# junghoseong/aircombat-selfplay

Hardware: AMD Instinct MI355X
Metric: agent-steps/sec (higher is better)
Workload: dtype f32

## Files before the change

### aircombat-selfplay_amd/csrc/aircombat.hip

```cpp
#include <hip/hip_runtime.h>
#include <stdint.h>
#include <stdio.h>
#include <string.h>
#include <string>
#include <vector>
#include <cmath>
#include <algorithm>
#include <chrono>
#include "../../include/aircombat.h"
#include "../../include/aircombat_buffer.h"
#include "clk_stamps.hpp"
#include "f16_device.hpp"
#include "f16_split.hpp"

using f16::State;
using f16::Derived;
using f16::Tab;
using f16::clampf;

#define AC_F_FIELDS(X)                                                                                           \
  X(vx) X(vy) X(vz) X(q0) X(q1) X(q2) X(q3) X(wp) X(wq) X(wr) X(hv1x) X(hv1y) X(hv1z) X(hv2x) X(hv2y) X(hv2z)   \
  X(ha1x) X(ha1y) X(ha1z) X(wdx) X(wdy) X(wdz) X(aix) X(aiy) X(aiz) X(bax) X(bay) X(baz) X(da) X(de) X(dr)       \
  X(thr) X(pin_r) X(pin_p) X(pin_y) X(pi_r) X(pi_p) X(pi_y) X(tef) X(ail) X(elev) X(sbdeg) X(alpha) X(mach)      \
  X(qc) X(vg) X(ap) X(aq) X(ar) X(npx) X(npy) X(npz) X(n1) X(n2) X(n2norm) X(ff) X(tank0) X(tank1)
// ... 734 lines not shown
    AC_CLKW(0, 120); AC_CLKW(1, 121); AC_CLKW(2, 122);
    __syncthreads();
  } else if (QUAD) {
    const int role = __builtin_amdgcn_readfirstlane(threadIdx.x >> 6);
    TableCopy<256> tc;
    tc.issue(P.tab);
    s = State{}; t = Task{};
    if (role == 0) { load_flight_role<0>(P.F, P.I, P.D, N, nn, s); t.status = state_word(P.F, SW_status, N, nn); }
    else if (role == 1) load_flight_role<1>(P.F, P.I, P.D, N, nn, s);
    else if (role == 2) { load_flight_role<2>(P.F, P.I, P.D, N, nn, s); t.status = state_word(P.F, SW_status, N, nn); }
    else {
      load_task(P.F, P.I, N, nn, t);
      s.ticks = state_word(P.F, SW_ticks, N, nn);
#pragma unroll
      for (int k = 0; k < MSLOTS; ++k) pre_st[k] = P.MI[((size_t)k * NMI + MI_status) * (size_t)N + nn];
    }
    __builtin_amdgcn_s_barrier();
    tc.write(lds_tab);
    a4 = make_float4(0.f, 0.f, 0.f, 0.f);
    __builtin_amdgcn_s_waitcnt(0x0F70);
    if (role == 1) arow.issue(act, c.act_dim);
    __syncthreads();
    if (role == 0) { quad_dynamics_wave(P, c, T, LQ, l, n, live, s, t); return; }
    if (role != 3 && split_helper_wave<true>(s, t, T, LQ.S, l, c.substeps, nullptr, nullptr, &arow)) return;
  } else if (PAIR) {
    const bool flight_role = __builtin_amdgcn_readfirstlane(threadIdx.x >> 6) == 1;
    PairFlightIn fin;
    if (!flight_role) {
      a4 = make_float4(0.f, 0.f, 0.f, 0.f);
      s = State{}; load_task(P.F, P.I, N, nn, t);
#pragma unroll
      for (int k = 0; k < MSLOTS; ++k) pre_st[k] = P.MI[((size_t)k * NMI + MI_status) * (size_t)N + nn];
    }
    stage_tables<128>(lds_tab, P.tab);
    if (flight_role) {
      pair_flight_load(P, c, nn, fin);
      pair_flight_wave<true>(P, c, T, LP, l, n, live, fin);
      return;
    }

  } else {
    TableCopy<64> tc;
    tc.issue(P.tab);
    a4 = load_controls(act, c.act_dim);
    if (TASK == AC_TASK_SHOOT_MISSILE) shoot_raw = act[4];
    load_state(P.F, P.I, P.D, N, nn, s, t);
    tc.commit(lds_tab);
  }
  AC_CLK(1);
  const Task was = t;
  constexpr bool OBS_BY_KIN = SPLIT && TASK == AC_TASK_SINGLECOMBAT;
  if (SPLIT) {
    const int role = __builtin_amdgcn_readfirstlane(threadIdx.x >> 6);
    if (split_helper_wave(s, t, T, L, l, c.substeps, nullptr, nullptr, &arow)) {
      if (OBS_BY_KIN && role == 1) {
        using namespace mail;
        wg_sync();
        Props q;
        q.alt_m = L.M[T_PR][l]; q.ub = L.M[T_PR + 5][l];
        q.n = L.M[T_PR + 9][l]; q.e = L.M[T_PR + 10][l]; q.u = L.M[T_PR + 11][l];
        q.vn = L.M[T_PR + 12][l]; q.ve = L.M[T_PR + 13][l]; q.vd = L.M[T_PR + 14][l];
        const Enemy Eq = exchange_1v1(q);
        L.M[T_RALT][l] = altitude_raw(q, c);
        L.M[T_RPOS][l] = posture_raw(q, Eq);
        wg_sync();
      }
      if (OBS_BY_KIN && role == 2) {
        using namespace mail;
        wg_sync();
        Props q;
        q.alt_m = L.M[T_PR][l]; q.sphi = L.M[T_PR + 1][l]; q.cphi = L.M[T_PR + 2][l]; q.stht = L.M[T_PR + 3][l]; q.ctht = L.M[T_PR + 4][l];
        q.ub = L.M[T_PR + 5][l]; q.vb = L.M[T_PR + 6][l]; q.wb = L.M[T_PR + 7][l]; q.vc = L.M[T_PR + 8][l];
        q.n = L.M[T_PR + 9][l]; q.e = L.M[T_PR + 10][l]; q.u = L.M[T_PR + 11][l];
        q.vn = L.M[T_PR + 12][l]; q.ve = L.M[T_PR + 13][l]; q.vd = L.M[T_PR + 14][l];
        const Enemy Eq = exchange_1v1(q);
        const Incoming none{false, 0, 0, 0, 0, 0, 0};
        float obq[OBS];
        observe_1v1<TASK>(q, Eq, none, obq);
        wg_sync();
        if (L.M[T_DONE][l] != 0.0f) {
          const float* tobs = (const float*)(P.tF + (size_t)NSW * 2) + slot * OBS;
#pragma unroll
          for (int k = 0; k < OBS; ++k) obq[k] = tobs[k];
        }
        float* row = lds_out + l * OBS;
#pragma unroll
        for (int k = 0; k < OBS; ++k) row[k] = obq[k];
        emit_obs_rows(P, lds_out, OBS, l);
      }
      return;
    }
  }
  Msl ms[MSLOTS];
  int nslots = 0, msl_was_active = 0;
  if (HAS_MSL) {
    nslots = min(c.num_missiles[slot], MSLOTS);
#pragma unroll
    for (int k = 0; k < MSLOTS; ++k) {
      const int st = (k < nslots) ? (PAIR ? pre_st[k] : P.MI[((size_t)k * NMI + MI_status) * (size_t)N + nn]) : MSL_INACTIVE;
      if (st != MSL_INACTIVE) { load_msl(P.MF, P.MI, N, nn, k, ms[k]); msl_was_active |= 1 << k; }
      else { ms[k] = Msl{}; ms[k].status = MSL_INACTIVE; }
    }
  }

  t.cur_step += 1;
  if (!SPLIT) {
    s.da = clampf(-1.0f, a4.x / 20.0f - 1.0f, 1.0f);
    s.de = clampf(-1.0f, a4.y / 20.0f - 1.0f, 1.0f);
    s.dr = clampf(-1.0f, a4.z / 20.0f - 1.0f, 1.0f);
    s.thr = clampf(0.0f, a4.w / 58.0f + 0.4f, 0.9f);
  }
  if (TASK == AC_TASK_SHOOT_MISSILE && !PAIR) t.shoot_action = (shoot_raw != 0.0f) ? 1 : 0;

  const MslParam MP = aim9l();
  bool have_pose = false;
  int last_tick = -1;
  bool env_has_missiles = false;
  if (PAIR) {
    bool mine = false;
#pragma unroll
    for (int k = 0; k < MSLOTS; ++k) mine = mine || ms[k].status != MSL_INACTIVE;
    const int other = __shfl_xor((int)mine, 1);
    env_has_missiles = mine || (bool)other;
  }
  int quad_nrun = 0;
  const int quad_ticks0 = s.ticks;
  for (int sub = 0; sub < c.substeps; ++sub) {
    bool fly_munitions = HAS_MSL;
    if (QUAD) {
      quad_substep_begin<true>(t, LQ, l, sub, env_has_missiles, quad_ticks0, quad_nrun, pr, c);
      fly_munitions = env_has_missiles;
    } else if (PAIR) {
      AC_CLK(2 + 8 * sub);
      pair_substep<true>(t, LP, l, sub, env_has_missiles, pr, c);
      AC_CLK(4 + 8 * sub);
      if (!env_has_missiles) continue;
    } else if (SPLIT) {
      if (dynamics_wave_tick(s, t, d, T, L, l, sub)) { have_pose = true; last_tick = sub; }
    } else if (t.status == AC_ALIVE) {
      if (t.bloods <= 0.0f) t.status = AC_SHOTDOWN;
      f16::tick<false>(s, d, T);
      have_pose = true;
    }
    if (HAS_MSL && fly_munitions) {
      if (!PAIR) {
      f16::locate(s, d);
      if (!have_pose) { f16::body_frame(s, d); have_pose = true; }
      make_props(s, d, c, pr);
      }
      float tx = __shfl_xor(pr.n, 1), ty = __shfl_xor(pr.e, 1), tz = __shfl_xor(pr.u, 1);
      float tvx = __shfl_xor(pr.vn, 1), tvy = __shfl_xor(pr.ve, 1), tvz = __shfl_xor(pr.vd, 1);
      bool talive = __shfl_xor(t.status, 1) == AC_ALIVE;
      bool hit_now = false;
#pragma unroll
      for (int k = 0; k < MSLOTS; ++k) {
        if (k < nslots && ms[k].status != MSL_INACTIVE) {
          missile_run(ms[k], MP, tx, ty, tz, tvx, tvy, tvz, talive, c);
          if (ms[k].status == MSL_HIT && talive) { hit_now = true; talive = false; }
        }
      }
      if (__shfl_xor((int)hit_now, 1) && t.status == AC_ALIVE) t.status = AC_SHOTDOWN;
      AC_CLK(5 + 8 * sub);
    }
    if (QUAD) wg_sync();
  }
  const bool split_located = SPLIT && dynamics_wave_finish(s, d, L, l, last_tick, c.substeps);
  if (PAIR) {
    if (QUAD) wg_sync();
    wg_sync();
    pair_read_final(LP, l, s, d, pr);
  } else if (!HAS_MSL || c.substeps == 0) {
    if (!split_located) f16::locate(s, d);
    if (!have_pose) f16::body_frame(s, d);
    make_props(s, d, c, pr);
  }
  AC_CLK(52);
  if (OBS_BY_KIN) {
    using namespace mail;
    L.M[T_PR][l] = pr.alt_m; L.M[T_PR + 1][l] = pr.sphi; L.M[T_PR + 2][l] = pr.cphi; L.M[T_PR + 3][l] = pr.stht; L.M[T_PR + 4][l] = pr.ctht;
    L.M[T_PR + 5][l] = pr.ub; L.M[T_PR + 6][l] = pr.vb; L.M[T_PR + 7][l] = pr.wb; L.M[T_PR + 8][l] = pr.vc;
    L.M[T_PR + 9][l] = pr.n; L.M[T_PR + 10][l] = pr.e; L.M[T_PR + 11][l] = pr.u;
    L.M[T_PR + 12][l] = pr.vn; L.M[T_PR + 13][l] = pr.ve; L.M[T_PR + 14][l] = pr.vd;
    wg_sync();
  }
  Enemy E = exchange_1v1(pr);

  if (c.use_artillery) {
    Geo g = ao_ta_r<false>(pr.n, pr.e, pr.u, pr.vn, pr.ve, pr.vd, E.n, E.e, E.u, E.vn, E.ve, E.vd);
    bool ealive = __shfl_xor(t.status, 1) == AC_ALIVE;
    float of = (g.AO <= 0.5236f) ? 1.0f - g.AO / 0.5236f : 0.0f;
    float Rk = g.R * 0.001f;
    float df = (Rk <= 1.0f) ? 1.0f : ((Rk <= 3.0f) ? (3.0f - Rk) * 0.5f : 0.0f);
    float dmg = ealive ? of * df : 0.0f;
    t.bloods -= __shfl_xor(dmg, 1);
  }
  if (HAS_MSL) {
    bool launch;
    if (TASK == AC_TASK_SHOOT_MISSILE && PAIR) t.shoot_action = ((QUAD ? LQ.S.M[mail::F_BITS][l] : LP.FIN[pair::FIN_BITS][l]) != 0.0f) ? 1 : 0;
    if (TASK == AC_TASK_DODGE_MISSILE) {
      const float dx = E.n - pr.n, dy = E.e - pr.e, dz = E.u - pr.u;
      const float dist = sqrtf(dx * dx + dy * dy + dz * dz);
      const float sp = sqrtf(pr.vn * pr.vn + pr.ve * pr.ve + pr.vd * pr.vd);
      const float ang = 57.29577951f * acosf(clampf(-1.0f, (dx * pr.vn + dy * pr.ve + dz * pr.vd) / (dist * sp + 1e-8f), 1.0f));
      const int len = c.lock_len;
      const unsigned bit = 1u << (unsigned)(t.lock_pos % len);
      t.lock_bits = (ang < c.max_attack_angle) ? (t.lock_bits | (int)bit) : (t.lock_bits & ~(int)bit);
      t.lock_pos += 1;
      const bool locked = __popc((unsigned)t.lock_bits & ((1u << len) - 1u)) >= len;
      launch = t.status == AC_ALIVE && locked && dist <= c.max_attack_distance && t.remaining > 0 &&
               (t.cur_step - t.last_shoot_time) >= c.min_attack_interval;
      if (launch) t.last_shoot_time = t.cur_step;
    } else {
      bool prev_done = t.last_missile < 0;
#pragma unroll
      for (int k = 0; k < MSLOTS; ++k)
        if (k == t.last_missile) prev_done = (ms[k].status == MSL_HIT || ms[k].status == MSL_MISS);
      launch = t.status == AC_ALIVE && t.shoot_action && t.remaining > 0 && prev_done;
    }
    int k = nslots - t.remaining;
// ... 1547 lines not shown
```

### aircombat-selfplay_amd/csrc/f16_split.hpp

```cpp
#pragma once

namespace f16 {
struct Surf { float aileron_rad, flaperon_rad, elevator_rad, rudder_rad, lef_rad, sb_rad, throttle_pos; };
struct DynVars {
  float gx, gy, gz;
  Atmos A;
  float mass, cgx, cgy, cgz, Jxx, Jyy, Jzz, Jxy, Jxz, Jyz;
  float vt, alpha, beta, ca, sa, cb, sb, qbar, mach, vg, qc, npx, npy, npz;
  float c00, c01, c02, c11, c12, c22, idet, im_;
  float bi2vel, ci2vel, qS, clb, cnb, cndr_m, kge;
  float4 g0, g1, g2, g3, ge, g7, m0, m1;
};
#define F16_DYN_REFS(k)                                                                                                          \
  float &gx = k.gx, &gy = k.gy, &gz = k.gz; Atmos& A = k.A;                                                                      \
  float &mass = k.mass, &cgx = k.cgx, &cgy = k.cgy, &cgz = k.cgz, &Jxx = k.Jxx, &Jyy = k.Jyy, &Jzz = k.Jzz, &Jxy = k.Jxy, &Jxz = k.Jxz, &Jyz = k.Jyz; \
  float &c00 = k.c00, &c01 = k.c01, &c02 = k.c02, &c11 = k.c11, &c12 = k.c12, &c22 = k.c22, &idet = k.idet, &im_ = k.im_; \
  float &vt = k.vt, &alpha = k.alpha, &beta = k.beta, &ca = k.ca, &sa = k.sa, &cb = k.cb, &sb = k.sb, &qbar = k.qbar, &mach = k.mach, &vg = k.vg,    \
        &qc = k.qc, &npx = k.npx, &npy = k.npy, &npz = k.npz;                                                                    \
  float &bi2vel = k.bi2vel, &ci2vel = k.ci2vel, &qS = k.qS, &clb = k.clb, &cnb = k.cnb, &cndr_m = k.cndr_m, &kge = k.kge; \
  float4 &g0 = k.g0, &g1 = k.g1, &g2 = k.g2, &g3 = k.g3, &ge = k.ge, &g7 = k.g7, &m0 = k.m0, &m1 = k.m1;                     \
  (void)gx; (void)gy; (void)gz; (void)A; (void)mass; (void)cgx; (void)cgy; (void)cgz; (void)Jxx; (void)Jyy; (void)Jzz; (void)Jxy; (void)Jxz; (void)Jyz; \
  (void)c00; (void)c01; (void)c02; (void)c11; (void)c12; (void)c22; (void)idet; (void)im_; \
  (void)vt; (void)alpha; (void)beta; (void)ca; (void)sa; (void)cb; (void)sb; (void)qbar; (void)mach; (void)vg; (void)qc; (void)npx; (void)npy; (void)npz; \
  (void)bi2vel; (void)ci2vel; (void)qS; (void)clb; (void)cnb; (void)cndr_m; (void)kge; (void)g0; (void)g1; (void)g2; (void)g3; (void)ge; (void)g7; (void)m0; (void)m1
// ... 179 lines not shown
    m1 = lerp4(rm2, rm3, fmach);
    cndr_m = lerpf(rn0, rn1, fmach);
    float hb = d.h_sl_ft * (1.0f / (float)F16_WINGSPAN);
    kge = 1.0f;
    if (hb < 1.1f) {
      constexpr float kGX[] = {0.0f, 0.1f, 0.15f, 0.2f, 0.3f, 0.4f, 0.5f, 0.6f, 0.7f, 0.8f, 0.9f, 1.0f, 1.1f};
      int ig = seg_index(kGX, hb);
      kge = lerpf(T[P_KCLGE_Y_OFF + ig - 1], T[P_KCLGE_Y_OFF + ig], seg_frac(T[P_KCLGE_X_OFF + ig - 1], T[P_KCLGE_X_OFF + ig], hb));
    }
  }
}

__device__ __forceinline__ void dyn_p4(State& s, Derived& d, DynVars& k, const Surf& sf, float thrust) {
  F16_DYN_REFS(k);
  const float aileron_rad = sf.aileron_rad, flaperon_rad = sf.flaperon_rad, rudder_rad = sf.rudder_rad, lef_rad = sf.lef_rad, sb_rad = sf.sb_rad;
  const float bw = (float)F16_WINGSPAN, cbar = (float)F16_CHORD;
  const float* Tb = d.T;
  (void)Tb;
  float tx = kInch2Ft * (cgx - (float)F16_THRUSTER_X), ty = kInch2Ft * ((float)F16_THRUSTER_Y - cgy), tz = kInch2Ft * (cgz - (float)F16_THRUSTER_Z);
  (void)tx;
  const float Mpy = tz * thrust, Mpz = -ty * thrust;

  float Fx, Fy, Fz, Mx, My, Mz;
  {
    float p = d.p, q = d.q, r = d.r;
    float qc = q * ci2vel;
    float CD = ge.x + m0.x + lef_rad * g0.x + flaperon_rad * (float)F16_K_CDDFLAPS + (float)F16_K_CDGEAR + sb_rad * g3.x +
               qc * (g0.y + lef_rad * g0.z);
    float CY = beta * ((float)F16_K_CYB + m0.y) + aileron_rad * (float)F16_K_CYDA + rudder_rad * (float)F16_K_CYDR +
               bi2vel * (p * g1.x + r * g1.y);
    float CL = kge * (ge.y + lef_rad * g0.w + flaperon_rad * (float)F16_K_CLDFLAPS + sb_rad * g3.y + qc * g2.x) + qc * sb_rad * g3.z;
    float Cl = clb + beta * m0.z + bi2vel * (p * g1.z + r * g1.w) + aileron_rad * (g7.x + alpha * m0.w) + rudder_rad * (g7.y + alpha * m1.x);
    float Cm = ge.z + alpha * m1.y + sb_rad * g3.w + qc * g2.y;
    float Cn = cnb + beta * m1.z + bi2vel * (p * g2.z + r * g2.w) + aileron_rad * (m1.w + g7.z) + rudder_rad * (g7.w + alpha * cndr_m);
    float D = qS * CD, Y = qS * CY, L = qS * CL;
    Fx = ca * cb * (-D) - ca * sb * Y + sa * L;
    Fy = sb * (-D) + cb * Y;
    Fz = sa * cb * (-D) - sa * sb * Y - ca * L;
    float ax = kInch2Ft * (cgx - (float)F16_AERORP_X), ay = kInch2Ft * ((float)F16_AERORP_Y - cgy), az = kInch2Ft * (cgz - (float)F16_AERORP_Z);
    Mx = qS * bw * Cl + (ay * Fz - az * Fy);
    My = qS * cbar * Cm + (az * Fx - ax * Fz);
    Mz = qS * bw * Cn + (ax * Fy - ay * Fx);
  }
  {
    float Tx = Fx + thrust, Ty = Fy, Tz = Fz;
    float Lm = Mx, Mm = My + Mpy, Nm = Mz + Mpz;
    float hx = Jxx * s.wp + Jxy * s.wq + Jxz * s.wr;
    float hy = Jxy * s.wp + Jyy * s.wq + Jyz * s.wr;
    float hz = Jxz * s.wp + Jyz * s.wq + Jzz * s.wr;
    float rx_ = Lm - (s.wq * hz - s.wr * hy), ry_ = Mm - (s.wr * hx - s.wp * hz), rz_ = Nm - (s.wp * hy - s.wq * hx);
    s.wdx = (c00 * rx_ + c01 * ry_ + c02 * rz_) * idet;
    s.wdy = (c01 * rx_ + c11 * ry_ + c12 * rz_) * idet;
    s.wdz = (c02 * rx_ + c12 * ry_ + c22 * rz_) * idet;
    s.bax = Tx * im_; s.bay = Ty * im_; s.baz = Tz * im_;
    s.aix = Tb[0] * s.bax + Tb[3] * s.bay + Tb[6] * s.baz + gx;
    s.aiy = Tb[1] * s.bax + Tb[4] * s.bay + Tb[7] * s.baz + gy;
    s.aiz = Tb[2] * s.bax + Tb[5] * s.bay + Tb[8] * s.baz + gz;
  }
  s.alpha = alpha; s.mach = mach; s.qc = qc; s.vg = vg;
  s.ap = d.p; s.aq = d.q; s.ar = d.r;
  s.npx = npx; s.npy = npy; s.npz = npz;
}

__device__ __forceinline__ void sys_fcs(State& s, float cthcph, float vbody, Surf& sf) {
  float &aileron_rad = sf.aileron_rad, &flaperon_rad = sf.flaperon_rad, &elevator_rad = sf.elevator_rad, &rudder_rad = sf.rudder_rad,
        &lef_rad = sf.lef_rad, &sb_rad = sf.sb_rad, &throttle_pos = sf.throttle_pos;
  const float alpha_p = s.alpha, mach_p = s.mach, qc_p = s.qc;
  float tef_rad = (qc_p < kQc250) ? 0.349f : ((mach_p > 0.9f) ? -0.0349f : 0.0f);
  s.tef = tef_kinematic(s.tef, 2.864789f * tef_rad);
  float roll_err = s.da - 0.31821f * s.ap;
  float roll_pid = pid(roll_err, s.pin_r, s.pi_r, qc_p < kQc20, 3.0f, 0.0005f, -0.00125f);
  float roll_cmd = clampf(-1.0f, roll_pid + s.da, 1.0f);
  aileron_rad = 0.375f * roll_cmd;
  s.ail = slew(s.ail, roll_cmd, -1.0f, 1.0f, 2.0f / 0.3f);
  constexpr float kAilX[] = C_FCS_AILERON_SPEED_COMPENSATED_X, kAilY[] = C_FCS_AILERON_SPEED_COMPENSATED_Y;
  float ail_sc = s.ail * tabc(kAilX, kAilY, mach_p);
  flaperon_rad = 1.4324f * (clampf(-1.0f, -s.tef - ail_sc, 1.0f) + clampf(-1.0f, s.tef - ail_sc, 1.0f));
  float elev_lim = clampf(-1.0f, s.de, 0.44f);
  constexpr float kElX[] = C_FCS_ELEVATOR_SCHEDULER_X, kElY[] = C_FCS_ELEVATOR_SCHEDULER_Y;
  float elev_sched = elev_lim * tabc(kElX, kElY, alpha_p);
  float pitch_err = elev_sched + 6.2f * s.aq - 0.020f * (s.npz - cthcph);
  float g_pid = clampf(-1.0f, pid(pitch_err, s.pin_p, s.pi_p, qc_p < kQc5, 0.3f, 0.025f, 0.0f), 1.0f);
  float pitch_sched = clampf(-1.0f, elev_sched + 1.0472f * alpha_p + g_pid, 1.0f);
  s.elev = slew(s.elev, pitch_sched, -1.0f, 1.0f, 2.0f / 0.3f);
  elevator_rad = 0.436f * s.elev;
  constexpr float kYwX[] = C_FCS_YAW_RATE_NORM_X, kYwY[] = C_FCS_YAW_RATE_NORM_Y;
  float yaw_err = s.dr + s.ar * tabc(kYwX, kYwY, s.vg) + 0.25f * s.npy;
  float yaw_pid = clampf(-1.0f, pid(yaw_err, s.pin_y, s.pi_y, qc_p < kQc10, 0.1055f, 0.00001f, 0.00005f), 1.0f);
  float yaw_sched = clampf(-1.0f, s.dr + yaw_pid, 1.0f);
  rudder_rad = 0.524f * slew(yaw_pid, yaw_sched, -1.0f, 1.0f, 2.0f / 0.4f);
  lef_rad = (alpha_p > 0.0873f) ? 0.262f : ((mach_p > 0.9f) ? -0.0349f : 0.0f);
  throttle_pos = 2.0f * s.thr;
  float sb_in = ((alpha_p * 57.29577951f >= 53.0f) && (vbody <= 18.0f)) ? 0.71667f * 60.0f : 0.0f;
  s.sbdeg = slew(s.sbdeg, sb_in, 0.0f, 60.0f, 60.0f);
  sb_rad = s.sbdeg * 0.01745329252f;

}

__device__ __forceinline__ void sys_mass(const State& s, DynVars& k) {
  F16_DYN_REFS(k);
  float fuel = s.tank0 + s.tank1;
  float weight = (float)F16_EMPTYWT + (float)F16_PM0_WEIGHT + fuel;
  mass = kLb2Slug * weight;
  float iw = 1.0f / weight;
  cgx = ((float)(F16_EMPTYWT * F16_CG_X + F16_PM0_WEIGHT * F16_PM0_X) + (float)F16_TANK0_X * fuel) * iw;
  cgy = ((float)F16_TANK0_Y * s.tank0 + (float)F16_TANK1_Y * s.tank1) * iw;
// ... 100 lines not shown
```

### aircombat-selfplay_amd/csrc/split_kernel.hpp

```cpp
#pragma once

namespace mail {
enum { RUNF,
       CTH, VB,
       MACH, QBAR, RHO, TEMP, HSL, ALPHA, BETA, QC, VG, NPY, NPZ, AP, AQ, AR,
       S_AIL, S_FLAP, S_ELEV, S_RUD, S_LEF, S_SB,
       THRUST,
       LK_CLB, LK_CNB, LK_G7,
       MASS0 = LK_G7 + 4, MASS_N = 18,
       F_TEF = MASS0 + MASS_N, F_PINR, F_PINP, F_PINY, F_PIR, F_PIP, F_PIY, F_AIL, F_ELEV, F_SBDEG, F_N1, F_N2, F_N2NORM, F_FF, F_TANK0, F_TANK1,
       F_ENG, F_DA, F_DE, F_DR, F_THR,
       F_BITS,
       K_W, K_V = K_W + 3,
       K_OUT = K_V + 3, K_OUT_N = 27,
       G_Q = K_OUT + K_OUT_N,
       G_H = G_Q + 8, G_NED = G_H + 1,
       QP_F = G_NED + 8, QP_F_N = 9,
       T_PR = QP_F + 2 * QP_F_N, T_PR_N = 15,
       T_DONE = T_PR + T_PR_N,
       T_RALT = T_DONE + 1, T_RPOS,
       ROWS = T_RPOS + 1 };
enum { GD_R, GD_X = GD_R + 6, GD_LAT = GD_X + 3, GD_QP = GD_LAT + 4, DROWS = GD_QP + 6 };
}
__device__ __forceinline__ void post_kin(float (*M)[64], int l, const f16::KinOut& o) {
  const float v[mail::K_OUT_N] = {o.T[0], o.T[1], o.T[2], o.T[3], o.T[4], o.T[5], o.T[6], o.T[7], o.T[8], o.h_sl_ft, o.n_eci[0], o.n_eci[1], o.n_eci[2],
                                  o.e_eci[0], o.e_eci[1], o.d_eci[0], o.d_eci[1], o.d_eci[2], o.gx, o.gy, o.gz, o.rxf, o.ryf, o.A.T, o.A.P, o.A.rho, o.A.a};
#pragma unroll
  for (int i = 0; i < mail::K_OUT_N; ++i) M[mail::K_OUT + i][l] = v[i];
}
__device__ __forceinline__ void fetch_kin(float (*M)[64], int l, f16::KinOut& o) {
  float v[mail::K_OUT_N];
#pragma unroll
  for (int i = 0; i < mail::K_OUT_N; ++i) v[i] = M[mail::K_OUT + i][l];
#pragma unroll
  for (int i = 0; i < 9; ++i) o.T[i] = v[i];
  o.h_sl_ft = v[9]; o.n_eci[0] = v[10]; o.n_eci[1] = v[11]; o.n_eci[2] = v[12]; o.e_eci[0] = v[13]; o.e_eci[1] = v[14];
  o.d_eci[0] = v[15]; o.d_eci[1] = v[16]; o.d_eci[2] = v[17]; o.gx = v[18]; o.gy = v[19]; o.gz = v[20]; o.rxf = v[21]; o.ryf = v[22];
  o.A.T = v[23]; o.A.P = v[24]; o.A.rho = v[25]; o.A.a = v[26];
}
__device__ __forceinline__ void post_mass(float (*M)[64], int l, const f16::DynVars& k) {
  const float v[mail::MASS_N] = {k.mass, k.cgx, k.cgy, k.cgz, k.Jxx, k.Jyy, k.Jzz, k.Jxy, k.Jxz, k.Jyz, k.c00, k.c01, k.c02, k.c11, k.c12, k.c22, k.idet, k.im_};
#pragma unroll
  for (int i = 0; i < mail::MASS_N; ++i) M[mail::MASS0 + i][l] = v[i];
}
__device__ __forceinline__ void fetch_mass(float (*M)[64], int l, f16::DynVars& k) {
  float v[mail::MASS_N];
#pragma unroll
  for (int i = 0; i < mail::MASS_N; ++i) v[i] = M[mail::MASS0 + i][l];
  k.mass = v[0]; k.cgx = v[1]; k.cgy = v[2]; k.cgz = v[3]; k.Jxx = v[4]; k.Jyy = v[5]; k.Jzz = v[6]; k.Jxy = v[7]; k.Jxz = v[8]; k.Jyz = v[9];
  k.c00 = v[10]; k.c01 = v[11]; k.c02 = v[12]; k.c11 = v[13]; k.c12 = v[14]; k.c22 = v[15]; k.idet = v[16]; k.im_ = v[17];
}
__device__ __forceinline__ void wg_sync() {
  __builtin_amdgcn_fence(__ATOMIC_RELEASE, "workgroup");
  __builtin_amdgcn_s_barrier();
  __builtin_amdgcn_fence(__ATOMIC_ACQUIRE, "workgroup");
}
typedef float f32x4 __attribute__((ext_vector_type(4)));
struct ActionRow {
  f32x4 v;
  __device__ __forceinline__ void issue(const float* p) { asm volatile("global_load_dwordx4 %0, %1, off" : "=&v"(v) : "v"(p) : "memory"); }
  __device__ __forceinline__ void take() { asm volatile("s_waitcnt vmcnt(0)" : "+v"(v) : : "memory"); }
};
struct ActionWord {
  float v;
  __device__ __forceinline__ void issue(const float* p) { asm volatile("global_load_dword %0, %1, off" : "=&v"(v) : "v"(p) : "memory"); }
  __device__ __forceinline__ void take() { asm volatile("s_waitcnt vmcnt(0)" : "+v"(v) : : "memory"); }
};
struct ActionFetch {
  ActionRow idx, bits;
  ActionWord bit;
  int extra;
  __device__ __forceinline__ void issue(const float* act, int act_dim) {
    extra = act_dim == 8 ? 4 : (act_dim == 5 ? 1 : 0);
    idx.issue(act);
// ... 35 lines not shown
      f16::sys_fcs(s, M[CTH][l], M[VB][l], sf);
      M[S_AIL][l] = sf.aileron_rad; M[S_FLAP][l] = sf.flaperon_rad; M[S_ELEV][l] = sf.elevator_rad;
      M[S_RUD][l] = sf.rudder_rad;  M[S_LEF][l] = sf.lef_rad;       M[S_SB][l] = sf.sb_rad;
    }
    AC_CLKW(1, 65 + sub * 8);
    wg_sync();
    if (run) {
      f16::Atmos A{};
      A.rho = M[RHO][l]; A.T = M[TEMP][l];
      const float mach = M[MACH][l], alpha = M[ALPHA][l], h_sl = M[HSL][l];
      float thrust;
      f16::sys_engine(s, T, mach, M[QBAR][l], A, h_sl, sf.throttle_pos, thrust);
      M[THRUST][l] = thrust;
    }
    AC_CLKW(1, 66 + sub * 8);
    wg_sync();
    if (run) {
      s.alpha = M[ALPHA][l]; s.mach = M[MACH][l]; s.qc = M[QC][l]; s.vg = M[VG][l];
      s.npy = M[NPY][l]; s.npz = M[NPZ][l]; s.ap = M[AP][l]; s.aq = M[AQ][l]; s.ar = M[AR][l];
      f16::sys_mass(s, km);
      post_mass(M, l, km);
    }
  }
  if (substeps == 0 && (row || raw)) {
    f32x4 v;
    if (row) { row->take(); v = row->idx.v; } else { v.x = raw->x; v.y = raw->y; v.z = raw->z; v.w = raw->w; }
    s.da = f16::clampf(-1.0f, v.x / 20.0f - 1.0f, 1.0f); s.de = f16::clampf(-1.0f, v.y / 20.0f - 1.0f, 1.0f);
    s.dr = f16::clampf(-1.0f, v.z / 20.0f - 1.0f, 1.0f); s.thr = f16::clampf(0.0f, v.w / 58.0f + 0.4f, 0.9f);
  }
  M[F_TEF][l] = s.tef; M[F_PINR][l] = s.pin_r; M[F_PINP][l] = s.pin_p; M[F_PINY][l] = s.pin_y;
  M[F_PIR][l] = s.pi_r; M[F_PIP][l] = s.pi_p; M[F_PIY][l] = s.pi_y; M[F_AIL][l] = s.ail; M[F_ELEV][l] = s.elev; M[F_SBDEG][l] = s.sbdeg;
  M[F_N1][l] = s.n1; M[F_N2][l] = s.n2; M[F_N2NORM][l] = s.n2norm; M[F_FF][l] = s.ff; M[F_TANK0][l] = s.tank0; M[F_TANK1][l] = s.tank1;
  M[F_ENG][l] = __int_as_float(s.eng);
  M[F_DA][l] = s.da; M[F_DE][l] = s.de; M[F_DR][l] = s.dr; M[F_THR][l] = s.thr;
  M[F_BITS][l] = row ? row->packed() : 0.0f;
  wg_sync();
}
__device__ __forceinline__ void post_quad_pose(float (*M)[64], double (*MD)[64], int l, int pb, const f16::State& s, int ticks, const DevCfg& c) {
  using namespace mail;
  f16::State sp{};
  sp.rx = s.rx; sp.ry = s.ry; sp.rz = s.rz; sp.ticks = ticks;
  f16::Derived dp;
  f16::locate(sp, dp);
  dp.vn = 0.0f; dp.ve = 0.0f; dp.vd = 0.0f;
  Props pp;
  make_pose(dp, c, pp);
  MD[GD_QP + 3 * pb][l] = pp.n64; MD[GD_QP + 3 * pb + 1][l] = pp.e64; MD[GD_QP + 3 * pb + 2][l] = pp.u64;
  const int r = QP_F + QP_F_N * pb;
  M[r][l] = pp.alt_m;
  M[r + 1][l] = dp.n_eci[0]; M[r + 2][l] = dp.n_eci[1]; M[r + 3][l] = dp.n_eci[2];
  M[r + 4][l] = dp.e_eci[0]; M[r + 5][l] = dp.e_eci[1];
  M[r + 6][l] = dp.d_eci[0]; M[r + 7][l] = dp.d_eci[1]; M[r + 8][l] = dp.d_eci[2];
}
template <bool QUAD = false, bool POSE = false>
__device__ __forceinline__ void kinematics_wave(f16::State& s, Task& t, const f16::Tab& T, float (*M)[64], double (*MD)[64], int l, int substeps,
                                                const DevCfg* cfg = nullptr) {
  using namespace mail;
  f16::KinOut o;
  const int ticks0 = s.ticks;
  const bool alive0 = t.status == AC_ALIVE && substeps > 0;
  if (alive0) { f16::kin_position(s, o); f16::kin_attitude(s, o); }
  if (QUAD) { MD[GD_R][l] = s.rx; MD[GD_R + 1][l] = s.ry; MD[GD_R + 2][l] = s.rz; }
  if (POSE) post_quad_pose(M, MD, l, 0, s, ticks0 + (alive0 ? 1 : 0), *cfg);
  for (int sub = 0; sub < substeps; ++sub) {
    AC_CLKW(2, 68 + sub * 8);
    wg_sync();
    const bool run = M[RUNF][l] != 0.0f;
    const bool last = sub + 1 == substeps;
    if (run) {
      const int pb = sub & 1;
      if (!QUAD) { MD[GD_R + 3 * pb][l] = s.rx; MD[GD_R + 3 * pb + 1][l] = s.ry; MD[GD_R + 3 * pb + 2][l] = s.rz; }
      M[G_Q + 4 * pb][l] = s.q0; M[G_Q + 4 * pb + 1][l] = s.q1; M[G_Q + 4 * pb + 2][l] = s.q2; M[G_Q + 4 * pb + 3][l] = s.q3;
    }
    if (run && !last) {
      s.wp = M[K_W][l]; s.wq = M[K_W + 1][l]; s.wr = M[K_W + 2][l];
      s.vx = M[K_V][l]; s.vy = M[K_V + 1][l]; s.vz = M[K_V + 2][l];
      f16::kin_position(s, o);
      if (QUAD) { const int nb = (sub + 1) & 1; MD[GD_R + 3 * nb][l] = s.rx; MD[GD_R + 3 * nb + 1][l] = s.ry; MD[GD_R + 3 * nb + 2][l] = s.rz; }
    } else if (run) {
      f16::Derived d;
      s.ticks += substeps;
      f16::locate(s, d);
      M[G_H][l] = d.h_sl_ft;
      M[G_NED][l] = d.n_eci[0]; M[G_NED + 1][l] = d.n_eci[1]; M[G_NED + 2][l] = d.n_eci[2];
      M[G_NED + 3][l] = d.e_eci[0]; M[G_NED + 4][l] = d.e_eci[1];
      M[G_NED + 5][l] = d.d_eci[0]; M[G_NED + 6][l] = d.d_eci[1]; M[G_NED + 7][l] = d.d_eci[2];
      MD[GD_X][l] = d.X; MD[GD_X + 1][l] = d.Y; MD[GD_X + 2][l] = d.Z;
      MD[GD_LAT][l] = d.sLat64; MD[GD_LAT + 1][l] = d.cLat64; MD[GD_LAT + 2][l] = d.sLon64; MD[GD_LAT + 3][l] = d.cLon64;
    }
    AC_CLKW(2, 69 + sub * 8);
    wg_sync();
    if (run) {
      f16::DynVars kl{};
      f16::Derived dd{};
      dd.h_sl_ft = 1e6f;
      kl.alpha = M[ALPHA][l]; kl.beta = M[BETA][l]; kl.mach = M[MACH][l]; kl.vt = 1.0f;
      f16::dyn_p3(dd, T, kl, f16::Surf{});
      M[LK_CLB][l] = kl.clb; M[LK_CNB][l] = kl.cnb;
      M[LK_G7][l] = kl.g7.x; M[LK_G7 + 1][l] = kl.g7.y; M[LK_G7 + 2][l] = kl.g7.z; M[LK_G7 + 3][l] = kl.g7.w;
    }
    if (run && !last) {
      f16::kin_attitude(s, o);
      post_kin(M, l, o);
    }
    AC_CLKW(2, 70 + sub * 8);
    wg_sync();
    if (POSE && run && !last) post_quad_pose(M, MD, l, (sub + 1) & 1, s, ticks0 + sub + 2, *cfg);
  }
  wg_sync();
}
struct SplitLds {
  float M[mail::ROWS][64];
  double MD[mail::DROWS][64];
};
template <bool QUAD = false, bool POSE = false>
__device__ __forceinline__ bool split_helper_wave(f16::State& s, Task& t, const f16::Tab& T, SplitLds& L, int l, int substeps, const float4* raw = nullptr,
                                                  const DevCfg* cfg = nullptr, ActionFetch* row = nullptr) {
  const int role = __builtin_amdgcn_readfirstlane(threadIdx.x >> 6);
  if (role == 2) { kinematics_wave<QUAD, POSE>(s, t, T, L.M, L.MD, l, substeps, cfg); return true; }
  if (role == 1) { systems_wave(s, t, T, L.M, l, substeps, raw, row); return true; }
  return false;
}
template <bool QUAD = false>
__device__ __forceinline__ bool dynamics_wave_tick(f16::State& s, Task& t, f16::Derived& d, const f16::Tab& T, SplitLds& L, int l, int sub, bool* d_stale = nullptr) {
  using namespace mail;
  float (*M)[64] = L.M;
  double (*MD)[64] = L.MD;
  bool run = t.status == AC_ALIVE;
  if (!QUAD && run && t.bloods <= 0.0f) t.status = AC_SHOTDOWN;
  f16::DynVars k;
  AC_CLK(2 + sub * 8);
  if (!QUAD) M[RUNF][l] = run ? 1.0f : 0.0f;
  const float b_wp = s.wp, b_wq = s.wq, b_wr = s.wr, b_vx = s.vx, b_vy = s.vy, b_vz = s.vz, b_ax = s.ha1x, b_ay = s.ha1y, b_az = s.ha1z;
  const float b_h1x = s.hv1x, b_h1y = s.hv1y, b_h1z = s.hv1z, b_h2x = s.hv2x, b_h2y = s.hv2y, b_h2z = s.hv2z;
  const int b_ticks = s.ticks;
  if (QUAD && !run) { M[K_V][l] = s.vx; M[K_V + 1][l] = s.vy; M[K_V + 2][l] = s.vz; }
  if (run) {
    if (sub == 0) f16::dyn_p1(s, d, k);
    else {
      f16::KinOut o;
      fetch_kin(M, l, o);
      f16::dyn_p1_lite(s, d, k, o);
    }
    M[K_W][l] = s.wp; M[K_W + 1][l] = s.wq; M[K_W + 2][l] = s.wr;
    M[K_V][l] = s.vx; M[K_V + 1][l] = s.vy; M[K_V + 2][l] = s.vz;
    M[CTH][l] = d.T[6] * d.d_eci[0] + d.T[7] * d.d_eci[1] + d.T[8] * d.d_eci[2];
    M[VB][l] = d.v;
  }
  AC_CLK(3 + sub * 8);
  wg_sync();
  AC_CLK(4 + sub * 8);
  if (QUAD && run && M[RUNF][l] == 0.0f) {
    s.wp = b_wp; s.wq = b_wq; s.wr = b_wr; s.vx = b_vx; s.vy = b_vy; s.vz = b_vz; s.ha1x = b_ax; s.ha1y = b_ay; s.ha1z = b_az; s.ticks = b_ticks;
    s.hv1x = b_h1x; s.hv1y = b_h1y; s.hv1z = b_h1z; s.hv2x = b_h2x; s.hv2y = b_h2y; s.hv2z = b_h2z;
    t.status = AC_SHOTDOWN;
    run = false;
    if (d_stale) *d_stale = true;
  }
  if (run) {
    fetch_mass(M, l, k);
    if (sub == 0) f16::dyn_p2<false>(s, d, k);
    else f16::dyn_p2<true>(s, d, k);
    M[BETA][l] = k.beta;
    M[MACH][l] = k.mach; M[QBAR][l] = k.qbar; M[RHO][l] = k.A.rho; M[TEMP][l] = k.A.T; M[HSL][l] = d.h_sl_ft;
    M[ALPHA][l] = k.alpha; M[QC][l] = k.qc; M[VG][l] = k.vg; M[NPY][l] = k.npy; M[NPZ][l] = k.npz;
    M[AP][l] = d.p; M[AQ][l] = d.q; M[AR][l] = d.r;
  }
  AC_CLK(5 + sub * 8);
  wg_sync();
  AC_CLK(6 + sub * 8);
  f16::Surf sf{};
  if (run) {
    sf = f16::Surf{M[S_AIL][l], M[S_FLAP][l], M[S_ELEV][l], M[S_RUD][l], M[S_LEF][l], M[S_SB][l], 0.0f};
    f16::dyn_p3(d, T, k, sf);
  }
  AC_CLK(7 + sub * 8);
  wg_sync();
  AC_CLK(8 + sub * 8);
  if (run) {
    k.clb = M[LK_CLB][l]; k.cnb = M[LK_CNB][l];
    k.g7 = make_float4(M[LK_G7][l], M[LK_G7 + 1][l], M[LK_G7 + 2][l], M[LK_G7 + 3][l]);
    f16::dyn_p4(s, d, k, sf, M[THRUST][l]);
    if (sub > 0) {
      const int pb = sub & 1;
      s.rx = MD[GD_R + 3 * pb][l]; s.ry = MD[GD_R + 3 * pb + 1][l]; s.rz = MD[GD_R + 3 * pb + 2][l];
    }
  }
  return run;
}
__device__ __forceinline__ bool dynamics_wave_finish(f16::State& s, f16::Derived& d, SplitLds& L, int l, int last_tick, int substeps) {
  using namespace mail;
  float (*M)[64] = L.M;
  double (*MD)[64] = L.MD;
  AC_CLK(50);
  wg_sync();
  AC_CLK(51);
  s.tef = M[F_TEF][l]; s.pin_r = M[F_PINR][l]; s.pin_p = M[F_PINP][l]; s.pin_y = M[F_PINY][l];
  s.pi_r = M[F_PIR][l]; s.pi_p = M[F_PIP][l]; s.pi_y = M[F_PIY][l]; s.ail = M[F_AIL][l]; s.elev = M[F_ELEV][l]; s.sbdeg = M[F_SBDEG][l];
  s.n1 = M[F_N1][l]; s.n2 = M[F_N2][l]; s.n2norm = M[F_N2NORM][l]; s.ff = M[F_FF][l]; s.tank0 = M[F_TANK0][l]; s.tank1 = M[F_TANK1][l];
  s.eng = __float_as_int(M[F_ENG][l]);
  s.da = M[F_DA][l]; s.de = M[F_DE][l]; s.dr = M[F_DR][l]; s.thr = M[F_THR][l];
  if (last_tick >= 1) {
    const int pb = last_tick & 1;
    s.q0 = M[G_Q + 4 * pb][l]; s.q1 = M[G_Q + 4 * pb + 1][l]; s.q2 = M[G_Q + 4 * pb + 2][l]; s.q3 = M[G_Q + 4 * pb + 3][l];
  }
  if (last_tick < 0 || last_tick != substeps - 1) return false;
  d.X = MD[GD_X][l]; d.Y = MD[GD_X + 1][l]; d.Z = MD[GD_X + 2][l];
  d.sLat64 = MD[GD_LAT][l]; d.cLat64 = MD[GD_LAT + 1][l]; d.sLon64 = MD[GD_LAT + 2][l]; d.cLon64 = MD[GD_LAT + 3][l];
  d.h_sl_ft = M[G_H][l];
  d.n_eci[0] = M[G_NED][l]; d.n_eci[1] = M[G_NED + 1][l]; d.n_eci[2] = M[G_NED + 2][l];
  d.e_eci[0] = M[G_NED + 3][l]; d.e_eci[1] = M[G_NED + 4][l]; d.e_eci[2] = 0.0f;
  d.d_eci[0] = M[G_NED + 5][l]; d.d_eci[1] = M[G_NED + 6][l]; d.d_eci[2] = M[G_NED + 7][l];
  return true;
}
__device__ __forceinline__ bool dynamics_wave_ticks(f16::State& s, Task& t, f16::Derived& d, const f16::Tab& T, SplitLds& L, int l, int substeps,
                                                    int& nrun) {
  int last_tick = -1;
  nrun = 0;
  for (int sub = 0; sub < substeps; ++sub)
    if (dynamics_wave_tick(s, t, d, T, L, l, sub)) { last_tick = sub; nrun += 1; }
  const bool located = dynamics_wave_finish(s, d, L, l, last_tick, substeps);
  if (last_tick >= 0 && !located) { f16::locate(s, d); return true; }
  return located;
}
```

Before: 235.6 million.

## Move rotational moment and rate integration to kinematics wave in split kernel

Under a new KIN_ROT template flag, the split kernel gives the kinematics wave the roll/pitch/yaw moment computation, the angular acceleration solve and the angular rate integration. The dynamics wave now computes only forces and translation, and passes forces, Cm and the needed coefficients to the other wave through LDS rows. The aim is to shorten the critical path of the dynamics wave by spreading work across the three cooperating waves. In exchange there is more LDS traffic, extra coefficient loads, and a reuse of mailbox rows that a static_assert guards.

```diff
diff --git a/aircombat-selfplay_amd/csrc/aircombat.hip b/aircombat-selfplay_amd/csrc/aircombat.hip
--- a/aircombat-selfplay_amd/csrc/aircombat.hip
+++ b/aircombat-selfplay_amd/csrc/aircombat.hip
@@ -810,7 +810,7 @@
   constexpr bool OBS_BY_KIN = SPLIT && TASK == AC_TASK_SINGLECOMBAT;
   if (SPLIT) {
     const int role = __builtin_amdgcn_readfirstlane(threadIdx.x >> 6);
-    if (split_helper_wave(s, t, T, L, l, c.substeps, nullptr, nullptr, &arow)) {
+    if (split_helper_wave<false, false, true>(s, t, T, L, l, c.substeps, nullptr, nullptr, &arow)) {
       if (OBS_BY_KIN && role == 1) {
         using namespace mail;
         wg_sync();
@@ -894,7 +894,7 @@
       AC_CLK(4 + 8 * sub);
       if (!env_has_missiles) continue;
     } else if (SPLIT) {
-      if (dynamics_wave_tick(s, t, d, T, L, l, sub)) { have_pose = true; last_tick = sub; }
+      if (dynamics_wave_tick<false, true>(s, t, d, T, L, l, sub)) { have_pose = true; last_tick = sub; }
     } else if (t.status == AC_ALIVE) {
       if (t.bloods <= 0.0f) t.status = AC_SHOTDOWN;
       f16::tick<false>(s, d, T);
@@ -922,7 +922,7 @@
     }
     if (QUAD) wg_sync();
   }
-  const bool split_located = SPLIT && dynamics_wave_finish(s, d, L, l, last_tick, c.substeps);
+  const bool split_located = SPLIT && dynamics_wave_finish<true>(s, d, L, l, last_tick, c.substeps);
   if (PAIR) {
     if (QUAD) wg_sync();
     wg_sync();
diff --git a/aircombat-selfplay_amd/csrc/f16_split.hpp b/aircombat-selfplay_amd/csrc/f16_split.hpp
--- a/aircombat-selfplay_amd/csrc/f16_split.hpp
+++ b/aircombat-selfplay_amd/csrc/f16_split.hpp
@@ -255,6 +255,105 @@
     s.wdx = (c00 * rx_ + c01 * ry_ + c02 * rz_) * idet;
     s.wdy = (c01 * rx_ + c11 * ry_ + c12 * rz_) * idet;
     s.wdz = (c02 * rx_ + c12 * ry_ + c22 * rz_) * idet;
+    s.bax = Tx * im_; s.bay = Ty * im_; s.baz = Tz * im_;
+    s.aix = Tb[0] * s.bax + Tb[3] * s.bay + Tb[6] * s.baz + gx;
+    s.aiy = Tb[1] * s.bax + Tb[4] * s.bay + Tb[7] * s.baz + gy;
+    s.aiz = Tb[2] * s.bax + Tb[5] * s.bay + Tb[8] * s.baz + gz;
+  }
+  s.alpha = alpha; s.mach = mach; s.qc = qc; s.vg = vg;
+  s.ap = d.p; s.aq = d.q; s.ar = d.r;
+  s.npx = npx; s.npy = npy; s.npz = npz;
+}
+
+__device__ __forceinline__ void dyn_p1_vel(State& s, Derived& d, DynVars& k, const KinOut& o) {
+  constexpr float dt = 1.0f / 60.0f;
+    s.hv2x = s.hv1x; s.hv2y = s.hv1y; s.hv2z = s.hv1z;
+    s.hv1x = s.vx; s.hv1y = s.vy; s.hv1z = s.vz;
+    s.vx += dt * (1.5f * s.aix - 0.5f * s.ha1x);
+    s.vy += dt * (1.5f * s.aiy - 0.5f * s.ha1y);
+    s.vz += dt * (1.5f * s.aiz - 0.5f * s.ha1z);
+    s.ha1x = s.aix; s.ha1y = s.aiy; s.ha1z = s.aiz;
+    s.ticks += 1;
+  d.h_sl_ft = o.h_sl_ft; k.gx = o.gx; k.gy = o.gy; k.gz = o.gz; k.A = o.A;
+  const float rxf = o.rxf, ryf = o.ryf;
+  float* T = d.T;
+#pragma unroll
+  for (int i = 0; i < 9; ++i) T[i] = o.T[i];
+#pragma unroll
+  for (int i = 0; i < 3; ++i) { d.n_eci[i] = o.n_eci[i]; d.d_eci[i] = o.d_eci[i]; }
+  d.e_eci[0] = o.e_eci[0]; d.e_eci[1] = o.e_eci[1]; d.e_eci[2] = 0.0f;
+  const float om = (float)kOmega;
+  float rvx = s.vx + om * ryf, rvy = s.vy - om * rxf, rvz = s.vz;
+  d.u = T[0] * rvx + T[1] * rvy + T[2] * rvz;
+  d.v = T[3] * rvx + T[4] * rvy + T[5] * rvz;
+  d.w = T[6] * rvx + T[7] * rvy + T[8] * rvz;
+  d.vn = d.n_eci[0] * rvx + d.n_eci[1] * rvy + d.n_eci[2] * rvz;
+  d.ve = d.e_eci[0] * rvx + d.e_eci[1] * rvy;
+  d.vd = d.d_eci[0] * rvx + d.d_eci[1] * rvy + d.d_eci[2] * rvz;
+  d.veci = sqrtf(s.vx * s.vx + s.vy * s.vy + s.vz * s.vz);
+}
+__device__ __forceinline__ void dyn_body_rates(const State& s, Derived& d) {
+  const float om = (float)kOmega;
+  const float* T = d.T;
+  d.p = s.wp - om * T[2]; d.q = s.wq - om * T[5]; d.r = s.wr - om * T[8];
+}
+__device__ __forceinline__ void kin_rates(State& s) {
+  constexpr float dt = 1.0f / 60.0f;
+    s.wp = fmaf(dt, s.wdx, s.wp); s.wq = fmaf(dt, s.wdy, s.wq); s.wr = fmaf(dt, s.wdz, s.wr);
+}
+
+__device__ __forceinline__ void dyn_forces(const Derived& d, DynVars& k, const Surf& sf, float& Fx, float& Fy, float& Fz, float& Cm) {
+  F16_DYN_REFS(k);
+  const float aileron_rad = sf.aileron_rad, flaperon_rad = sf.flaperon_rad, rudder_rad = sf.rudder_rad, lef_rad = sf.lef_rad, sb_rad = sf.sb_rad;
+  {
+    float p = d.p, q = d.q, r = d.r;
+    float qc = q * ci2vel;
+    float CD = ge.x + m0.x + lef_rad * g0.x + flaperon_rad * (float)F16_K_CDDFLAPS + (float)F16_K_CDGEAR + sb_rad * g3.x +
+               qc * (g0.y + lef_rad * g0.z);
+    float CY = beta * ((float)F16_K_CYB + m0.y) + aileron_rad * (float)F16_K_CYDA + rudder_rad * (float)F16_K_CYDR +
+               bi2vel * (p * g1.x + r * g1.y);
+    float CL = kge * (ge.y + lef_rad * g0.w + flaperon_rad * (float)F16_K_CLDFLAPS + sb_rad * g3.y + qc * g2.x) + qc * sb_rad * g3.z;
+    Cm = ge.z + alpha * m1.y + sb_rad * g3.w + qc * g2.y;
+    float D = qS * CD, Y = qS * CY, L = qS * CL;
+    Fx = ca * cb * (-D) - ca * sb * Y + sa * L;
+    Fy = sb * (-D) + cb * Y;
+    Fz = sa * cb * (-D) - sa * sb * Y - ca * L;
+  }
+}
+__device__ __forceinline__ void kin_moments(State& s, const Derived& d, DynVars& k, const Surf& sf, float thrust, float Fx, float Fy, float Fz, float Cm) {
+  F16_DYN_REFS(k);
+  const float aileron_rad = sf.aileron_rad, rudder_rad = sf.rudder_rad;
+  const float bw = (float)F16_WINGSPAN, cbar = (float)F16_CHORD;
+  float tx = kInch2Ft * (cgx - (float)F16_THRUSTER_X), ty = kInch2Ft * ((float)F16_THRUSTER_Y - cgy), tz = kInch2Ft * (cgz - (float)F16_THRUSTER_Z);
+  (void)tx;
+  const float Mpy = tz * thrust, Mpz = -ty * thrust;
+
+  float Mx, My, Mz;
+  {
+    float p = d.p, r = d.r;
+    float Cl = clb + beta * m0.z + bi2vel * (p * g1.z + r * g1.w) + aileron_rad * (g7.x + alpha * m0.w) + rudder_rad * (g7.y + alpha * m1.x);
+    float Cn = cnb + beta * m1.z + bi2vel * (p * g2.z + r * g2.w) + aileron_rad * (m1.w + g7.z) + rudder_rad * (g7.w + alpha * cndr_m);
+    float ax = kInch2Ft * (cgx - (float)F16_AERORP_X), ay = kInch2Ft * ((float)F16_AERORP_Y - cgy), az = kInch2Ft * (cgz - (float)F16_AERORP_Z);
+    Mx = qS * bw * Cl + (ay * Fz - az * Fy);
+    My = qS * cbar * Cm + (az * Fx - ax * Fz);
+    Mz = qS * bw * Cn + (ax * Fy - ay * Fx);
+  }
+  {
+    float Lm = Mx, Mm = My + Mpy, Nm = Mz + Mpz;
+    float hx = Jxx * s.wp + Jxy * s.wq + Jxz * s.wr;
+    float hy = Jxy * s.wp + Jyy * s.wq + Jyz * s.wr;
+    float hz = Jxz * s.wp + Jyz * s.wq + Jzz * s.wr;
+    float rx_ = Lm - (s.wq * hz - s.wr * hy), ry_ = Mm - (s.wr * hx - s.wp * hz), rz_ = Nm - (s.wp * hy - s.wq * hx);
+    s.wdx = (c00 * rx_ + c01 * ry_ + c02 * rz_) * idet;
+    s.wdy = (c01 * rx_ + c11 * ry_ + c12 * rz_) * idet;
+    s.wdz = (c02 * rx_ + c12 * ry_ + c22 * rz_) * idet;
+  }
+}
+__device__ __forceinline__ void dyn_translation(State& s, Derived& d, DynVars& k, float thrust, float Fx, float Fy, float Fz) {
+  F16_DYN_REFS(k);
+  const float* Tb = d.T;
+  {
+    float Tx = Fx + thrust, Ty = Fy, Tz = Fz;
     s.bax = Tx * im_; s.bay = Ty * im_; s.baz = Tz * im_;
     s.aix = Tb[0] * s.bax + Tb[3] * s.bay + Tb[6] * s.baz + gx;
     s.aiy = Tb[1] * s.bax + Tb[4] * s.bay + Tb[7] * s.baz + gy;
diff --git a/aircombat-selfplay_amd/csrc/split_kernel.hpp b/aircombat-selfplay_amd/csrc/split_kernel.hpp
--- a/aircombat-selfplay_amd/csrc/split_kernel.hpp
+++ b/aircombat-selfplay_amd/csrc/split_kernel.hpp
@@ -19,7 +19,12 @@
        T_PR = QP_F + 2 * QP_F_N, T_PR_N = 15,
        T_DONE = T_PR + T_PR_N,
        T_RALT = T_DONE + 1, T_RPOS,
-       ROWS = T_RPOS + 1 };
+       ROWS = T_RPOS + 1,
+       R_F = QP_F, R_CM = R_F + 3, R_C = R_CM + 1,
+       R_W = R_C + 10,
+       R_VT = R_W + 3,
+       R_WD = LK_CLB };
+static_assert(R_VT < QP_F + 2 * QP_F_N && R_WD + 3 <= LK_G7 + 4, "KIN_ROT rows overlap rows that form uses");
 enum { GD_R, GD_X = GD_R + 6, GD_LAT = GD_X + 3, GD_QP = GD_LAT + 4, DROWS = GD_QP + 6 };
 }
 __device__ __forceinline__ void post_kin(float (*M)[64], int l, const f16::KinOut& o) {
@@ -161,7 +166,7 @@
   M[r + 4][l] = dp.e_eci[0]; M[r + 5][l] = dp.e_eci[1];
   M[r + 6][l] = dp.d_eci[0]; M[r + 7][l] = dp.d_eci[1]; M[r + 8][l] = dp.d_eci[2];
 }
-template <bool QUAD = false, bool POSE = false>
+template <bool QUAD = false, bool POSE = false, bool KIN_ROT = false>
 __device__ __forceinline__ void kinematics_wave(f16::State& s, Task& t, const f16::Tab& T, float (*M)[64], double (*MD)[64], int l, int substeps,
                                                 const DevCfg* cfg = nullptr) {
   using namespace mail;
@@ -181,8 +186,13 @@
       if (!QUAD) { MD[GD_R + 3 * pb][l] = s.rx; MD[GD_R + 3 * pb + 1][l] = s.ry; MD[GD_R + 3 * pb + 2][l] = s.rz; }
       M[G_Q + 4 * pb][l] = s.q0; M[G_Q + 4 * pb + 1][l] = s.q1; M[G_Q + 4 * pb + 2][l] = s.q2; M[G_Q + 4 * pb + 3][l] = s.q3;
     }
+    f16::DynVars kl{};
+    if (KIN_ROT && run) {
+      if (sub == 0) { s.wp = M[K_W][l]; s.wq = M[K_W + 1][l]; s.wr = M[K_W + 2][l]; }
+      fetch_mass(M, l, kl);
+    }
     if (run && !last) {
-      s.wp = M[K_W][l]; s.wq = M[K_W + 1][l]; s.wr = M[K_W + 2][l];
+      if (!KIN_ROT) { s.wp = M[K_W][l]; s.wq = M[K_W + 1][l]; s.wr = M[K_W + 2][l]; }
       s.vx = M[K_V][l]; s.vy = M[K_V + 1][l]; s.vz = M[K_V + 2][l];
       f16::kin_position(s, o);
       if (QUAD) { const int nb = (sub + 1) & 1; MD[GD_R + 3 * nb][l] = s.rx; MD[GD_R + 3 * nb + 1][l] = s.ry; MD[GD_R + 3 * nb + 2][l] = s.rz; }
@@ -200,13 +210,15 @@
     AC_CLKW(2, 69 + sub * 8);
     wg_sync();
     if (run) {
-      f16::DynVars kl{};
       f16::Derived dd{};
       dd.h_sl_ft = 1e6f;
       kl.alpha = M[ALPHA][l]; kl.beta = M[BETA][l]; kl.mach = M[MACH][l]; kl.vt = 1.0f;
+      if (KIN_ROT) { kl.vt = M[R_VT][l]; kl.qbar = M[QBAR][l]; }
       f16::dyn_p3(dd, T, kl, f16::Surf{});
-      M[LK_CLB][l] = kl.clb; M[LK_CNB][l] = kl.cnb;
-      M[LK_G7][l] = kl.g7.x; M[LK_G7 + 1][l] = kl.g7.y; M[LK_G7 + 2][l] = kl.g7.z; M[LK_G7 + 3][l] = kl.g7.w;
+      if (!KIN_ROT) {
+        M[LK_CLB][l] = kl.clb; M[LK_CNB][l] = kl.cnb;
+        M[LK_G7][l] = kl.g7.x; M[LK_G7 + 1][l] = kl.g7.y; M[LK_G7 + 2][l] = kl.g7.z; M[LK_G7 + 3][l] = kl.g7.w;
+      }
     }
     if (run && !last) {
       f16::kin_attitude(s, o);
@@ -214,6 +226,22 @@
     }
     AC_CLKW(2, 70 + sub * 8);
     wg_sync();
+    if (KIN_ROT && run) {
+      const float Fx = M[R_F][l], Fy = M[R_F + 1][l], Fz = M[R_F + 2][l], Cm = M[R_CM][l];
+      kl.m0.z = M[R_C][l]; kl.m0.w = M[R_C + 1][l]; kl.m1.x = M[R_C + 2][l]; kl.m1.z = M[R_C + 3][l]; kl.m1.w = M[R_C + 4][l];
+      kl.g1.z = M[R_C + 5][l]; kl.g1.w = M[R_C + 6][l]; kl.g2.z = M[R_C + 7][l]; kl.g2.w = M[R_C + 8][l]; kl.cndr_m = M[R_C + 9][l];
+      f16::Derived dr{};
+      dr.p = M[AP][l]; dr.r = M[AR][l];
+      f16::Surf sf{};
+      sf.aileron_rad = M[S_AIL][l]; sf.rudder_rad = M[S_RUD][l];
+      f16::kin_moments(s, dr, kl, sf, M[THRUST][l], Fx, Fy, Fz, Cm);
+      M[R_WD][l] = s.wdx; M[R_WD + 1][l] = s.wdy; M[R_WD + 2][l] = s.wdz;
+      if (!last) {
+        f16::kin_rates(s);
+        M[R_W][l] = s.wp; M[R_W + 1][l] = s.wq; M[R_W + 2][l] = s.wr;
+      }
+      AC_CLKW(2, 71 + sub * 8);
+    }
     if (POSE && run && !last) post_quad_pose(M, MD, l, (sub + 1) & 1, s, ticks0 + sub + 2, *cfg);
   }
   wg_sync();
@@ -222,15 +250,15 @@
   float M[mail::ROWS][64];
   double MD[mail::DROWS][64];
 };
-template <bool QUAD = false, bool POSE = false>
+template <bool QUAD = false, bool POSE = false, bool KIN_ROT = false>
 __device__ __forceinline__ bool split_helper_wave(f16::State& s, Task& t, const f16::Tab& T, SplitLds& L, int l, int substeps, const float4* raw = nullptr,
                                                   const DevCfg* cfg = nullptr, ActionFetch* row = nullptr) {
   const int role = __builtin_amdgcn_readfirstlane(threadIdx.x >> 6);
-  if (role == 2) { kinematics_wave<QUAD, POSE>(s, t, T, L.M, L.MD, l, substeps, cfg); return true; }
+  if (role == 2) { kinematics_wave<QUAD, POSE, KIN_ROT>(s, t, T, L.M, L.MD, l, substeps, cfg); return true; }
   if (role == 1) { systems_wave(s, t, T, L.M, l, substeps, raw, row); return true; }
   return false;
 }
-template <bool QUAD = false>
+template <bool QUAD = false, bool KIN_ROT = false>
 __device__ __forceinline__ bool dynamics_wave_tick(f16::State& s, Task& t, f16::Derived& d, const f16::Tab& T, SplitLds& L, int l, int sub, bool* d_stale = nullptr) {
   using namespace mail;
   float (*M)[64] = L.M;
@@ -249,9 +277,10 @@
     else {
       f16::KinOut o;
       fetch_kin(M, l, o);
-      f16::dyn_p1_lite(s, d, k, o);
-    }
-    M[K_W][l] = s.wp; M[K_W + 1][l] = s.wq; M[K_W + 2][l] = s.wr;
+      if (KIN_ROT) f16::dyn_p1_vel(s, d, k, o);
+      else f16::dyn_p1_lite(s, d, k, o);
+    }
+    if (!KIN_ROT || sub == 0) { M[K_W][l] = s.wp; M[K_W + 1][l] = s.wq; M[K_W + 2][l] = s.wr; }
     M[K_V][l] = s.vx; M[K_V + 1][l] = s.vy; M[K_V + 2][l] = s.vz;
     M[CTH][l] = d.T[6] * d.d_eci[0] + d.T[7] * d.d_eci[1] + d.T[8] * d.d_eci[2];
     M[VB][l] = d.v;
@@ -267,6 +296,10 @@
     if (d_stale) *d_stale = true;
   }
   if (run) {
+    if (KIN_ROT && sub > 0) {
+      s.wp = M[R_W][l]; s.wq = M[R_W + 1][l]; s.wr = M[R_W + 2][l]; s.wdx = M[R_WD][l]; s.wdy = M[R_WD + 1][l]; s.wdz = M[R_WD + 2][l];
+      f16::dyn_body_rates(s, d);
+    }
     fetch_mass(M, l, k);
     if (sub == 0) f16::dyn_p2<false>(s, d, k);
     else f16::dyn_p2<true>(s, d, k);
@@ -274,22 +307,34 @@
     M[MACH][l] = k.mach; M[QBAR][l] = k.qbar; M[RHO][l] = k.A.rho; M[TEMP][l] = k.A.T; M[HSL][l] = d.h_sl_ft;
     M[ALPHA][l] = k.alpha; M[QC][l] = k.qc; M[VG][l] = k.vg; M[NPY][l] = k.npy; M[NPZ][l] = k.npz;
     M[AP][l] = d.p; M[AQ][l] = d.q; M[AR][l] = d.r;
+    if (KIN_ROT) M[R_VT][l] = k.vt;
   }
   AC_CLK(5 + sub * 8);
   wg_sync();
   AC_CLK(6 + sub * 8);
   f16::Surf sf{};
+  float Fx = 0.0f, Fy = 0.0f, Fz = 0.0f;
   if (run) {
     sf = f16::Surf{M[S_AIL][l], M[S_FLAP][l], M[S_ELEV][l], M[S_RUD][l], M[S_LEF][l], M[S_SB][l], 0.0f};
     f16::dyn_p3(d, T, k, sf);
+    if (KIN_ROT) {
+      float Cm;
+      f16::dyn_forces(d, k, sf, Fx, Fy, Fz, Cm);
+      M[R_F][l] = Fx; M[R_F + 1][l] = Fy; M[R_F + 2][l] = Fz; M[R_CM][l] = Cm;
+      M[R_C][l] = k.m0.z; M[R_C + 1][l] = k.m0.w; M[R_C + 2][l] = k.m1.x; M[R_C + 3][l] = k.m1.z; M[R_C + 4][l] = k.m1.w;
+      M[R_C + 5][l] = k.g1.z; M[R_C + 6][l] = k.g1.w; M[R_C + 7][l] = k.g2.z; M[R_C + 8][l] = k.g2.w; M[R_C + 9][l] = k.cndr_m;
+    }
   }
   AC_CLK(7 + sub * 8);
   wg_sync();
   AC_CLK(8 + sub * 8);
   if (run) {
-    k.clb = M[LK_CLB][l]; k.cnb = M[LK_CNB][l];
-    k.g7 = make_float4(M[LK_G7][l], M[LK_G7 + 1][l], M[LK_G7 + 2][l], M[LK_G7 + 3][l]);
-    f16::dyn_p4(s, d, k, sf, M[THRUST][l]);
+    if (KIN_ROT) f16::dyn_translation(s, d, k, M[THRUST][l], Fx, Fy, Fz);
+    else {
+      k.clb = M[LK_CLB][l]; k.cnb = M[LK_CNB][l];
+      k.g7 = make_float4(M[LK_G7][l], M[LK_G7 + 1][l], M[LK_G7 + 2][l], M[LK_G7 + 3][l]);
+      f16::dyn_p4(s, d, k, sf, M[THRUST][l]);
+    }
     if (sub > 0) {
       const int pb = sub & 1;
       s.rx = MD[GD_R + 3 * pb][l]; s.ry = MD[GD_R + 3 * pb + 1][l]; s.rz = MD[GD_R + 3 * pb + 2][l];
@@ -297,6 +342,7 @@
   }
   return run;
 }
+template <bool KIN_ROT = false>
 __device__ __forceinline__ bool dynamics_wave_finish(f16::State& s, f16::Derived& d, SplitLds& L, int l, int last_tick, int substeps) {
   using namespace mail;
   float (*M)[64] = L.M;
@@ -309,6 +355,7 @@
   s.n1 = M[F_N1][l]; s.n2 = M[F_N2][l]; s.n2norm = M[F_N2NORM][l]; s.ff = M[F_FF][l]; s.tank0 = M[F_TANK0][l]; s.tank1 = M[F_TANK1][l];
   s.eng = __float_as_int(M[F_ENG][l]);
   s.da = M[F_DA][l]; s.de = M[F_DE][l]; s.dr = M[F_DR][l]; s.thr = M[F_THR][l];
+  if (KIN_ROT && last_tick >= 0) { s.wdx = M[R_WD][l]; s.wdy = M[R_WD + 1][l]; s.wdz = M[R_WD + 2][l]; }
   if (last_tick >= 1) {
     const int pb = last_tick & 1;
     s.q0 = M[G_Q + 4 * pb][l]; s.q1 = M[G_Q + 4 * pb + 1][l]; s.q2 = M[G_Q + 4 * pb + 2][l]; s.q3 = M[G_Q + 4 * pb + 3][l];
```

Measured after the change: 240.1 million, median of 6. 1.9% higher.
